# hir0shim/singleSpMV

Measured on AMD Instinct MI355X. Metric: SpMV GFLOP/s (fp64) + achieved HBM GB/s, higher is better.
Workload: dtype f64

## Files before the change

singlespmv_amd/csrc/k_bin.hip:

```cpp
#include "device.hpp"
#include "internal.hpp"

namespace spmv {

typedef uint32_t bin_u32x4 __attribute__((ext_vector_type(4)));

template <int U>
struct MulBatch {
    double v[U];
    uint32_t c[U];
    int32_t d[U];
};

template <int U, int PL, int MODE, bool LONG>
__device__ __forceinline__ void mul_load(MulBatch<U> &B, int64_t base, int64_t e0, int64_t e1, int lane,
                                         const double *__restrict__ val1, const uint16_t *__restrict__ cs1,
                                         const int32_t *__restrict__ dst1, int64_t ls, int64_t lsh,
                                         const int32_t *__restrict__ lcode) {
    if constexpr (!LONG) {
        const double *vb = val1 + base + lane;
        const uint16_t *cb = cs1 + base + lane;
        const int32_t *db = dst1 + ((base + lane) >> PL);
#pragma unroll
        for (int u = 0; u < U; ++u) {
            B.v[u] = ld_stream(vb + u * 64);
            B.c[u] = (uint32_t)__builtin_nontemporal_load(cb + u * 64);
            if constexpr ((MODE & 4) == 0) B.d[u] = ld_stream(db + u * (64 >> PL));
        }
        (void)e0;
        (void)e1;
        (void)ls;
        (void)lsh;
        (void)lcode;
        (void)db;
    } else {
#pragma unroll
        for (int u = 0; u < U; ++u) {
            const int64_t e = base + u * 64 + lane;
            const int64_t ee = e < e1 ? e : e0;
            B.v[u] = ld_stream(val1 + ee);
            B.c[u] = (uint32_t)__builtin_nontemporal_load(cs1 + ee);
            if (base + u * 64 >= ls) B.d[u] = ld_stream(lcode + (e < e1 ? e + lsh : 0));
            else if constexpr ((MODE & 4) == 0) B.d[u] = ld_stream(dst1 + (ee >> PL));
        }
    }
}

__device__ __forceinline__ void mul_long_block(double pr, int32_t code, bool ok, int lane,
                                               double *__restrict__ prod) {
    const bool start = code < 0 || !ok;
    const uint64_t starts = __ballot(start);
    const uint64_t upto = starts & (~0ull >> (63 - lane));
    const int seg = 63 - __clzll((long long)upto);
    const int r16 = lane & 15, row = lane >> 4;
    double v = ok ? pr : 0.0, t;
    t = dpp_f64<0x111, 0xF>(v);
    if (r16 >= 1 && lane - 1 >= seg) v = __dadd_rn(t, v);
    t = dpp_f64<0x112, 0xF>(v);
    if (r16 >= 2 && lane - 2 >= seg) v = __dadd_rn(t, v);
    t = dpp_f64<0x114, 0xF>(v);
    if (r16 >= 4 && lane - 4 >= seg) v = __dadd_rn(t, v);
    t = dpp_f64<0x118, 0xF>(v);
    if (r16 >= 8 && lane - 8 >= seg) v = __dadd_rn(t, v);
    t = dpp_f64<0x142, 0xA>(v);
    if ((row & 1) && seg <= row * 16 - 1) v = __dadd_rn(t, v);
    t = dpp_f64<0x143, 0xC>(v);
    if (row >= 2 && seg <= 31) v = __dadd_rn(t, v);
    const int32_t pos = code & 0x7FFFFFFF;
    if (ok && pos != 0x7FFFFFFF) prod[pos] = v;
}

template <int U, int MODE, int PL, bool LONG>
__device__ __forceinline__ void mul_store(const MulBatch<U> &B, int64_t base, int64_t e1, int lane,
                                          const double *xs, double *__restrict__ prod, int64_t ls) {
#pragma unroll
    for (int u = 0; u < U; ++u) {
        const int64_t e = base + u * 64 + lane;
        if (LONG && base + u * 64 >= ls) {
            mul_long_block(__dmul_rn(B.v[u], xs[B.c[u]]), B.d[u], e < e1, lane, prod);
        } else if (e < e1) {
            const double pr = __dmul_rn(B.v[u], xs[B.c[u]]);
            double *dp = (MODE & 4) ? prod + e : prod + ((int64_t)B.d[u] << PL) + (e & ((1 << PL) - 1));
            if (MODE & 1) __builtin_nontemporal_store(pr, dp);
            else *dp = pr;
        }
    }
}

template <int U, int MODE, int PL, bool LONG>
__global__ __launch_bounds__(kBinMulThreads) void bin_mul_kernel(
    const int64_t *__restrict__ piece_off, int64_t q_base, const int32_t *__restrict__ piece_strip,
    const int64_t *__restrict__ piece_begin, const int64_t *__restrict__ piece_end,
    const double *__restrict__ val1, const uint16_t *__restrict__ cs1, const int32_t *__restrict__ dst1,
    const double *__restrict__ x, int64_t n, int32_t strip, double *__restrict__ prod,
    const int64_t *__restrict__ lstart, const int64_t *__restrict__ lshift, const int32_t *__restrict__ lcode,
    int32_t xburst) {
    __shared__ double xs[kBinMaxStrip];
    constexpr int NW = kBinMulThreads / 64;
    constexpr int64_t STEP = (int64_t)NW * 64 * U;
    const int w = __builtin_amdgcn_readfirstlane(threadIdx.x >> 6);
    const int lane = threadIdx.x & 63;
    const int64_t q0 = piece_off[q_base + blockIdx.x], q1 = piece_off[q_base + blockIdx.x + 1];
    for (int64_t q = q0; q < q1; ++q) {
        const int32_t st = piece_strip[q];
        const int64_t c0 = (int64_t)st * strip;
        const int64_t e0 = piece_begin[q], e1 = piece_end[q];
        const int64_t ls = LONG ? lstart[st] : INT64_MAX, lsh = LONG ? lshift[st] : 0;
        const int cw = (int)(n - c0 < strip ? n - c0 : strip);
        __syncthreads();
        constexpr int XL = 8;
        if constexpr ((MODE & 256) != 0) {
            const int full = cw & ~127;
            for (int k = w; k * 128 < full; k += NW)
                __builtin_amdgcn_global_load_lds(
                    (const __attribute__((address_space(1))) void *)(x + c0 + k * 128 + lane * 2),
                    (__attribute__((address_space(3))) void *)(xs + k * 128), 16, 0, 0);
            for (int i = full + threadIdx.x; i < cw; i += kBinMulThreads) xs[i] = x[c0 + i];
            __builtin_amdgcn_s_waitcnt(0x0F70);
        } else if (LONG || !xburst) {
            for (int i = threadIdx.x; i < cw; i += kBinMulThreads) xs[i] = x[c0 + i];
        } else for (int i0 = threadIdx.x; i0 < cw; i0 += XL * kBinMulThreads) {
            double t[XL];
#pragma unroll
            for (int k = 0; k < XL; ++k) {
                const int i = i0 + k * kBinMulThreads;
                t[k] = i < cw ? x[c0 + i] : 0.0;
            }
#pragma unroll
            for (int k = 0; k < XL; ++k) {
                const int i = i0 + k * kBinMulThreads;
                if (i < cw) xs[i] = t[k];
            }
        }
        __syncthreads();
        const int64_t first = e0 + (int64_t)w * 64 * U;
        const int64_t nit = first < e1 ? (e1 - first + STEP - 1) / STEP : 0;
        auto bat = [&](int64_t j) { return first + j * STEP; };
        MulBatch<U> A, B;
        if (nit > 0) mul_load<U, PL, MODE, LONG>(A, bat(0), e0, e1, lane, val1, cs1, dst1, ls, lsh, lcode);
        for (int64_t it = 0; it < nit; it += 2) {
            const int64_t ba = bat(it), bb = bat(it + 1);
            if (it + 1 < nit) mul_load<U, PL, MODE, LONG>(B, bb, e0, e1, lane, val1, cs1, dst1, ls, lsh, lcode);
            mul_store<U, MODE, PL, LONG>(A, ba, e1, lane, xs, prod, ls);
            if (it + 1 < nit) {
                if (it + 2 < nit)
                    mul_load<U, PL, MODE, LONG>(A, bat(it + 2), e0, e1, lane, val1, cs1, dst1, ls, lsh, lcode);
                mul_store<U, MODE, PL, LONG>(B, bb, e1, lane, xs, prod, ls);
            }
        }
    }
}

template <int U>
struct SumBatch {
    double v[U];
    uint32_t w[U / 2];
    __device__ __forceinline__ uint32_t slot(int u) const { return (w[u >> 1] >> (16 * (u & 1))) & 0xFFFFu; }
};

template <int U>
__device__ __forceinline__ void sum_load(SumBatch<U> &B, int64_t base, int lane, int64_t pbase, int64_t sbase,
                                         const uint16_t *__restrict__ slot2, const double *__restrict__ prod) {
    static_assert(U % 8 == 0, "slots are read 8 per 16-byte load");
    const bin_u32x4 *sp = reinterpret_cast<const bin_u32x4 *>(slot2 + sbase + (int64_t)lane * 8);
#pragma unroll
    for (int q = 0; q < U / 8; ++q) {
        const bin_u32x4 w = __builtin_nontemporal_load(sp + q * 64);
#pragma unroll
        for (int h = 0; h < 4; ++h) B.w[4 * q + h] = w[h];
    }
    const double *pp = prod + (base - pbase) + lane;
#pragma unroll
    for (int u = 0; u < U; ++u) B.v[u] = ld_stream(pp + u * 64);
}

template <int U>
__device__ __forceinline__ void sum_add(const SumBatch<U> &B, double *ys) {
#pragma unroll
    for (int u = 0; u < U; ++u) atomicAdd(&ys[B.slot(u)], B.v[u]);
}

template <int W2, int U>
__global__ __launch_bounds__(64 * W2) void bin_sum_kernel(
    int64_t b0, int64_t b1, int64_t nbins, int64_t nblk, const int64_t *__restrict__ run_off,
    const int64_t *__restrict__ srun_off, const int32_t *__restrict__ bin_row0, int64_t pbase,
    const uint16_t *__restrict__ slot2,
    const double *__restrict__ prod, double *__restrict__ y) {
    constexpr int SLICE = kBinLdsDoubles / W2;
    constexpr int64_t STEP = 64 * U;
    __shared__ double ylds[kBinLdsDoubles];
    const int w = __builtin_amdgcn_readfirstlane(threadIdx.x >> 6);
    const int lane = threadIdx.x & 63;
    double *ys = ylds + w * SLICE;
    const int64_t bfirst = b0 + (int64_t)blockIdx.x * W2 + w, bstride = (int64_t)gridDim.x * W2;
    if (bfirst >= b1) return;
    int64_t cb = bfirst, k = 0, pos = run_off[cb], end = run_off[cb + 1], rs = pos, ss = srun_off[cb];
    auto next = [&](int64_t &lo, int64_t &sb, int64_t &bb) -> bool {
        while (pos >= end) {
            if (++k >= nblk) {
                cb += bstride;
                if (cb >= b1) return false;
                k = 0;
                pos = rs = run_off[cb];
                end = run_off[cb + 1];
                ss = srun_off[cb];
                continue;
            }
            pos = rs = run_off[k * nbins + cb];
            end = run_off[k * nbins + cb + 1];
            ss = srun_off[k * nbins + cb];
        }
        lo = pos;
        sb = ss + (lo - rs);
        bb = cb;
        pos = pos + STEP < end ? pos + STEP : end;
        return true;
    };
    int64_t acc = -1, done = bfirst;
    auto write_zero = [&](int64_t bz) {
        const int64_t r0 = bin_row0[bz];
        const int rows = (int)(bin_row0[bz + 1] - r0);
        for (int i = lane; i < rows; i += 64) __builtin_nontemporal_store(0.0, y + r0 + i);
    };
    auto finish = [&]() {
        const int64_t r0 = bin_row0[acc];
        const int rows = (int)(bin_row0[acc + 1] - r0);
        __builtin_amdgcn_fence(__ATOMIC_SEQ_CST, "wavefront");
        for (int i = lane; i < rows; i += 64) __builtin_nontemporal_store(ys[i], y + r0 + i);
        __builtin_amdgcn_fence(__ATOMIC_SEQ_CST, "wavefront");
        done = acc + bstride;
    };
    auto begin = [&](int64_t nb) {
        if (nb == acc) return;
        if (acc >= 0) finish();
        for (; done < nb; done += bstride) write_zero(done);
        const int rows = (int)(bin_row0[nb + 1] - bin_row0[nb]);
        for (int i = lane; i < rows; i += 64) ys[i] = 0.0;
        acc = nb;
        done = nb + bstride;
    };
    SumBatch<U> A, B;
    int64_t alo, asb, ab, blo, bsb, bbn;
    bool has_a = next(alo, asb, ab);
    if (has_a) sum_load<U>(A, alo, lane, pbase, asb, slot2, prod);
    while (has_a) {
        const bool has_b = next(blo, bsb, bbn);
        if (has_b) sum_load<U>(B, blo, lane, pbase, bsb, slot2, prod);
        begin(ab);
        sum_add<U>(A, ys);
        if (!has_b) break;
        has_a = next(alo, asb, ab);
        if (has_a) sum_load<U>(A, alo, lane, pbase, asb, slot2, prod);
        begin(bbn);
        sum_add<U>(B, ys);
    }
    if (acc >= 0) finish();
    for (; done < b1; done += bstride) write_zero(done);
}

template <int U>
struct SumTab {
    int32_t t[U / 8];
};

template <int U>
__device__ __forceinline__ void sum_mo_tab(SumTab<U> &T, int64_t sb, int lane, const int32_t *__restrict__ mtab) {
    static_assert(U == 32, "U/8 = 4 table words per lane: one 16-byte load");
    const bin_u32x4 w = __builtin_nontemporal_load(reinterpret_cast<const bin_u32x4 *>(mtab + (sb >> 3)) + lane);
#pragma unroll
    for (int h = 0; h < 4; ++h) T.t[h] = (int32_t)w[h];
}

template <int U>
__device__ __forceinline__ void sum_mo_load(SumBatch<U> &B, const SumTab<U> &T, int64_t sb, int lane,
                                            const uint16_t *__restrict__ slot2, const double *__restrict__ prod) {
    const bin_u32x4 *sp = reinterpret_cast<const bin_u32x4 *>(slot2 + sb + (int64_t)lane * 8);
#pragma unroll
    for (int q = 0; q < U / 8; ++q) {
        const bin_u32x4 w = __builtin_nontemporal_load(sp + q * 64);
#pragma unroll
        for (int h = 0; h < 4; ++h) B.w[4 * q + h] = w[h];
    }
    const double *pl = prod + (lane & 7);
    int c[U];
#pragma unroll
    for (int u = 0; u < U; ++u) c[u] = __builtin_amdgcn_ds_bpermute((((u & 7) << 3) + (lane >> 3)) << 2, T.t[u >> 3]);
    __builtin_amdgcn_sched_barrier(0);
#pragma unroll
    for (int u = 0; u < U; ++u) B.v[u] = pl[c[u]];
}

template <int W2, int U>
__global__ __launch_bounds__(64 * W2) void bin_sum_bin_kernel(
    int64_t b0, int64_t b1, const int64_t *__restrict__ run_off, const int64_t *__restrict__ srun_off,
    const int32_t *__restrict__ bin_row0, const uint16_t *__restrict__ slot2, const int32_t *__restrict__ mtab,
    const double *__restrict__ prod, double *__restrict__ y) {
    constexpr int SLICE = kBinLdsDoubles / W2;
    constexpr int64_t STEP = 64 * U;
    __shared__ double ylds[kBinLdsDoubles];
    const int w = __builtin_amdgcn_readfirstlane(threadIdx.x >> 6);
    const int lane = threadIdx.x & 63;
    double *ys = ylds + w * SLICE;
    struct BinRun {
        int64_t r0 = 0, nb = 0, ss0 = 0;
        int rows = 0;
        __device__ int64_t s(int64_t j) const { return ss0 + j * STEP; }
    };
    auto bin_at = [&](int64_t b) {
        BinRun R;
        R.r0 = bin_row0[b];
        R.rows = (int)(bin_row0[b + 1] - R.r0);
        R.ss0 = srun_off[b];
        R.nb = (run_off[b + 1] - run_off[b] + STEP - 1) / STEP;
        return R;
    };
    const int64_t bstride = (int64_t)gridDim.x * W2;
    int64_t b = b0 + (int64_t)blockIdx.x * W2 + w;
    if (b >= b1) return;
    BinRun R = bin_at(b);
    for (int i = lane; i < R.rows; i += 64) ys[i] = 0.0;
    SumBatch<U> PA, PB;
    SumTab<U> TA, TB;
    bool pre = false;
    for (;;) {
        const int64_t bn = b + bstride;
        const bool more = bn < b1;
        const BinRun N = more ? bin_at(bn) : R;
        const bool pfn = more && N.nb > 0;
        auto sbat = [&](int64_t j) -> int64_t {
            if (j < R.nb) return R.s(j);
            return pfn ? N.s(j - R.nb < N.nb ? j - R.nb : N.nb - 1) : R.s(R.nb - 1);
        };
        bool swapped = false;
        if (R.nb > 0) {
            if (!pre) {
                sum_mo_tab<U>(TA, sbat(0), lane, mtab);
                sum_mo_tab<U>(TB, sbat(1), lane, mtab);
                sum_mo_load<U>(PA, TA, sbat(0), lane, slot2, prod);
            } else if (R.nb == 1) {
                sum_mo_tab<U>(TB, sbat(1), lane, mtab);
            }
            for (int64_t j = 0;; j += 2) {
                sum_mo_tab<U>(TA, sbat(j + 2), lane, mtab);
                sum_mo_load<U>(PB, TB, sbat(j + 1), lane, slot2, prod);
                sum_add<U>(PA, ys);
                if (j + 1 >= R.nb) {
                    swapped = true;
                    break;
                }
                sum_mo_tab<U>(TB, sbat(j + 3), lane, mtab);
                sum_mo_load<U>(PA, TA, sbat(j + 2), lane, slot2, prod);
                sum_add<U>(PB, ys);
                if (j + 2 >= R.nb) break;
            }
        }
        pre = R.nb > 0 && pfn;
        __builtin_amdgcn_fence(__ATOMIC_SEQ_CST, "wavefront");
        for (int i = lane; i < R.rows; i += 64) __builtin_nontemporal_store(ys[i], y + R.r0 + i);
        __builtin_amdgcn_fence(__ATOMIC_SEQ_CST, "wavefront");
        if (!more) break;
        for (int i = lane; i < N.rows; i += 64) ys[i] = 0.0;
        if (pre && swapped) {
            PA = PB;
            TB = TA;
        }
        b = bn;
        R = N;
    }
}

template <int W2>
static void launch_sum_mo(const spmv_plan_s *p, double *y) {
    const BinDev &B = p->bin;
    hipLaunchKernelGGL((bin_sum_bin_kernel<W2, 32>), dim3((unsigned)B.nwg2), dim3(64 * W2), 0, p->stream,
                       (int64_t)0, B.n_bins, B.run_off, B.srun_off, B.bin_row0, B.slot2, B.mtab, B.prod, y);
}

template <int MODE, int PL, int U = 8>
static void launch_mul_t(const spmv_plan_s *p, int g, const double *x) {
    const BinDev &B = p->bin;
    if (B.long_len > 0)
        hipLaunchKernelGGL((bin_mul_kernel<U, MODE, PL, true>), dim3((unsigned)B.nwg1), dim3(kBinMulThreads), 0,
                           p->stream, B.piece_off, (int64_t)g * B.nwg1, B.piece_strip, B.piece_begin, B.piece_end,
                           B.val1, B.cs1, B.dst1, x, p->n, (int32_t)B.strip, B.prod, B.lstart, B.lshift, B.lcode,
                           B.xburst);
    else
        hipLaunchKernelGGL((bin_mul_kernel<U, MODE, PL, false>), dim3((unsigned)B.nwg1), dim3(kBinMulThreads), 0,
                           p->stream, B.piece_off, (int64_t)g * B.nwg1, B.piece_strip, B.piece_begin, B.piece_end,
                           B.val1, B.cs1, B.dst1, x, p->n, (int32_t)B.strip, B.prod, nullptr, nullptr, nullptr,
                           B.xburst);
}

template <int PL>
static void launch_mul_p(const spmv_plan_s *p, int g, const double *x) {
    bool dma = (reinterpret_cast<uintptr_t>(x) & 15) == 0 && p->bin.strip % 2 == 0;
    if (launch_dbg(p->bin.dbg) & (1 << 24)) dma = false;
    if (p->bin.mo) {
        if (dma) launch_mul_t<256 | 4, PL>(p, g, x);
        else launch_mul_t<4, PL>(p, g, x);
    } else {
        if (dma) launch_mul_t<256 | 1, PL>(p, g, x);
        else launch_mul_t<1, PL>(p, g, x);
    }
}

static void launch_mul(const spmv_plan_s *p, int g, const double *x) {
    if (p->bin.pad_log == 5) launch_mul_p<5>(p, g, x);
    else if (p->bin.pad_log == 4) launch_mul_p<4>(p, g, x);
    else launch_mul_p<3>(p, g, x);
}

template <int W2, int U>
static void launch_sum_w(const spmv_plan_s *p, int g, double *y) {
    const BinDev &B = p->bin;
    const int64_t b0 = g < 0 ? 0 : B.g_bin[g], b1 = g < 0 ? B.n_bins : B.g_bin[g + 1];
    const int64_t pbase = g < 0 ? 0 : B.g_prod[g];
    hipLaunchKernelGGL((bin_sum_kernel<W2, U>), dim3((unsigned)B.nwg2), dim3(64 * W2), 0, p->stream, b0, b1,
                       B.n_bins, B.n_blocks, B.run_off, B.srun_off, B.bin_row0, pbase, B.slot2, B.prod, y);
}

int bin_time_mul(const spmv_plan_s *p, const double *x, float *ms) {
    const BinDev &B = p->bin;
    hipEvent_t a, b;
    SPMV_HIP_TRY(hipEventCreate(&a));
    SPMV_HIP_TRY(hipEventCreate(&b));
    for (int rep = 0; rep < 2; ++rep) {
        if (rep == 1) SPMV_HIP_TRY(hipEventRecord(a, p->stream));
        for (int g = 0; g < B.G; ++g) {
            launch_mul(p, g, x);
        }
    }
    SPMV_HIP_TRY(hipEventRecord(b, p->stream));
    SPMV_HIP_TRY(hipEventSynchronize(b));
    SPMV_HIP_TRY(hipEventElapsedTime(ms, a, b));
    (void)hipEventDestroy(a);
    (void)hipEventDestroy(b);
    return SPMV_SUCCESS;
}

int launch_bin(const spmv_plan_s *p, const double *x, double *y) {
    const BinDev &B = p->bin;
    if (p->m == 0) return SPMV_SUCCESS;
    if (p->nnz == 0) {
        SPMV_HIP_TRY(hipMemsetAsync(y, 0, sizeof(double) * (size_t)p->m, p->stream));
        return SPMV_SUCCESS;
    }
    auto sum = [&](int g) {
        if (B.mo) {
            if (B.sum_waves == 2) launch_sum_mo<2>(p, y);
            else launch_sum_mo<4>(p, y);
            return;
        }
        if (B.sum_waves == 2) launch_sum_w<2, 32>(p, g, y);
        else if (B.sum_waves == 4) launch_sum_w<4, 32>(p, g, y);
        else launch_sum_w<8, 8>(p, g, y);
    };
    for (int g = 0; g < B.G; ++g) {
        launch_mul(p, g, x);
        SPMV_HIP_TRY(hipGetLastError());
        if (B.reuse) {
            phase_mark(p);
            sum(g);
            SPMV_HIP_TRY(hipGetLastError());
            if (g + 1 < B.G) phase_mark(p);
        }
    }
    if (!B.reuse) {
        phase_mark(p);
        sum(-1);
        SPMV_HIP_TRY(hipGetLastError());
    }
    return SPMV_SUCCESS;
}

}
```

Baseline: 396.4.

## Add team mode to bin sum kernel sharing one LDS bin across waves

Restructures the bin sum kernel so that, for the 2-wave configuration, P waves form a team working on one bin with a single LDS slice. The waves take turns applying atomic adds while the others prefetch their next batch, and the per-bin index tables are read through the constant address space. The aim is to overlap loads with LDS accumulation and to raise the number of resident workgroups by shrinking LDS per block. The cost is a workgroup barrier every turn, plus serialised adds within each team. The 4-wave setting keeps the old per-wave path (P=1), and probe flags allow switching between variants.

After: 396.7 (median of 3 runs). About the same (+0.1%).

```diff
diff --git a/singlespmv_amd/csrc/k_bin.hip b/singlespmv_amd/csrc/k_bin.hip
--- a/singlespmv_amd/csrc/k_bin.hip
+++ b/singlespmv_amd/csrc/k_bin.hip
@@ -180,22 +180,17 @@
     for (int u = 0; u < U; ++u) atomicAdd(&ys[B.slot(u)], B.v[u]);
 }
 
-template <int W2, int U>
-__global__ __launch_bounds__(64 * W2) void bin_sum_kernel(
-    int64_t b0, int64_t b1, int64_t nbins, int64_t nblk, const int64_t *__restrict__ run_off,
-    const int64_t *__restrict__ srun_off, const int32_t *__restrict__ bin_row0, int64_t pbase,
-    const uint16_t *__restrict__ slot2,
-    const double *__restrict__ prod, double *__restrict__ y) {
-    constexpr int SLICE = kBinLdsDoubles / W2;
-    constexpr int64_t STEP = 64 * U;
-    __shared__ double ylds[kBinLdsDoubles];
-    const int w = __builtin_amdgcn_readfirstlane(threadIdx.x >> 6);
-    const int lane = threadIdx.x & 63;
-    double *ys = ylds + w * SLICE;
-    const int64_t bfirst = b0 + (int64_t)blockIdx.x * W2 + w, bstride = (int64_t)gridDim.x * W2;
-    if (bfirst >= b1) return;
-    int64_t cb = bfirst, k = 0, pos = run_off[cb], end = run_off[cb + 1], rs = pos, ss = srun_off[cb];
-    auto next = [&](int64_t &lo, int64_t &sb, int64_t &bb) -> bool {
+template <typename TAB>
+struct SumCursor {
+    TAB run_off, srun_off;
+    int64_t nbins, nblk, b1, bstride;
+    int64_t cb, k, pos, end, rs, ss;
+    __device__ __forceinline__ SumCursor(TAB ro, TAB so, int64_t nbins_, int64_t nblk_, int64_t bfirst, int64_t b1_,
+                                         int64_t bstride_)
+        : run_off(ro), srun_off(so), nbins(nbins_), nblk(nblk_), b1(b1_), bstride(bstride_), cb(bfirst), k(0),
+          pos(ro[bfirst]), end(ro[bfirst + 1]), rs(pos), ss(so[bfirst]) {}
+    template <int64_t STEP>
+    __device__ __forceinline__ bool next(int64_t &lo, int64_t &sb, int64_t &bb) {
         while (pos >= end) {
             if (++k >= nblk) {
                 cb += bstride;
@@ -215,8 +210,90 @@
         bb = cb;
         pos = pos + STEP < end ? pos + STEP : end;
         return true;
-    };
+    }
+};
+
+template <int W2, int U, int P>
+__global__ __launch_bounds__(64 * (P == 1 ? W2 : P)) void bin_sum_kernel(
+    int64_t b0, int64_t b1, int64_t nbins, int64_t nblk, const int64_t *__restrict__ run_off,
+    const int64_t *__restrict__ srun_off, const int32_t *__restrict__ bin_row0, int64_t pbase,
+    const uint16_t *__restrict__ slot2,
+    const double *__restrict__ prod, double *__restrict__ y) {
+    constexpr int SLICE = kBinLdsDoubles / W2;
+    constexpr int64_t STEP = 64 * U;
+    __shared__ double ylds[P == 1 ? kBinLdsDoubles : SLICE];
+    const int w = __builtin_amdgcn_readfirstlane(threadIdx.x >> 6);
+    const int lane = threadIdx.x & 63;
+    double *ys = P == 1 ? ylds + w * SLICE : ylds;
+    const int64_t bfirst = b0 + (P == 1 ? (int64_t)blockIdx.x * W2 + w : (int64_t)blockIdx.x);
+    const int64_t bstride = (int64_t)gridDim.x * (P == 1 ? W2 : 1);
+    if (bfirst >= b1) return;
     int64_t acc = -1, done = bfirst;
+    if constexpr (P > 1) {
+        typedef const __attribute__((address_space(4))) int64_t *ctab;
+        const SumCursor<ctab> first((ctab)run_off, (ctab)srun_off, nbins, nblk, bfirst, b1, bstride);
+        SumCursor<ctab> step = first, mine = first;
+        constexpr int T = 64 * P;
+        const int tid = threadIdx.x;
+        auto team_barrier = [&]() {
+            __builtin_amdgcn_fence(__ATOMIC_SEQ_CST, "wavefront");
+            __builtin_amdgcn_s_waitcnt(0xC07F);
+            __builtin_amdgcn_s_barrier();
+            __builtin_amdgcn_fence(__ATOMIC_SEQ_CST, "wavefront");
+        };
+        auto zero_rows = [&](int64_t bz) {
+            const int64_t r0 = bin_row0[bz];
+            const int rows = (int)(bin_row0[bz + 1] - r0);
+            for (int i = tid; i < rows; i += T) __builtin_nontemporal_store(0.0, y + r0 + i);
+        };
+        auto write_back = [&]() {
+            const int64_t r0 = bin_row0[acc];
+            const int rows = (int)(bin_row0[acc + 1] - r0);
+            for (int i0 = tid; i0 < rows; i0 += 4 * T) {
+                double v[4];
+#pragma unroll
+                for (int q = 0; q < 4; ++q) v[q] = i0 + q * T < rows ? ys[i0 + q * T] : 0.0;
+#pragma unroll
+                for (int q = 0; q < 4; ++q)
+                    if (i0 + q * T < rows) __builtin_nontemporal_store(v[q], y + r0 + i0 + q * T);
+            }
+            done = acc + bstride;
+        };
+        SumBatch<U> A;
+        auto load_mine = [&](int skip) {
+            int64_t lo, sb, bb;
+            bool has = true;
+#pragma unroll
+            for (int i = 0; i < P - 1; ++i)
+                if (i < skip && has) has = mine.template next<STEP>(lo, sb, bb);
+            if (has && mine.template next<STEP>(lo, sb, bb)) sum_load<U>(A, lo, lane, pbase, sb, slot2, prod);
+        };
+        load_mine(w);
+        int turn = 0;
+        int64_t lo, sb, nb;
+        while (step.template next<STEP>(lo, sb, nb)) {
+            if (nb != acc) {
+                if (acc >= 0) write_back();
+                for (; done < nb; done += bstride) zero_rows(done);
+                const int rows = (int)(bin_row0[nb + 1] - bin_row0[nb]);
+                for (int i = tid; i < rows; i += T) ys[i] = 0.0;
+                acc = nb;
+                done = nb + bstride;
+                team_barrier();
+            }
+            if (turn == w) {
+                sum_add<U>(A, ys);
+                load_mine(P - 1);
+            }
+            team_barrier();
+            turn = turn + 1 == P ? 0 : turn + 1;
+        }
+        if (acc >= 0) write_back();
+        for (; done < b1; done += bstride) zero_rows(done);
+        return;
+    }
+    SumCursor<const int64_t *> cur(run_off, srun_off, nbins, nblk, bfirst, b1, bstride);
+    auto next = [&](int64_t &lo, int64_t &sb, int64_t &bb) -> bool { return cur.template next<STEP>(lo, sb, bb); };
     auto write_zero = [&](int64_t bz) {
         const int64_t r0 = bin_row0[bz];
         const int rows = (int)(bin_row0[bz + 1] - r0);
@@ -410,13 +487,36 @@
     else launch_mul_p<3>(p, g, x);
 }
 
-template <int W2, int U>
+template <int W2, int U, int P>
 static void launch_sum_w(const spmv_plan_s *p, int g, double *y) {
     const BinDev &B = p->bin;
     const int64_t b0 = g < 0 ? 0 : B.g_bin[g], b1 = g < 0 ? B.n_bins : B.g_bin[g + 1];
     const int64_t pbase = g < 0 ? 0 : B.g_prod[g];
-    hipLaunchKernelGGL((bin_sum_kernel<W2, U>), dim3((unsigned)B.nwg2), dim3(64 * W2), 0, p->stream, b0, b1,
-                       B.n_bins, B.n_blocks, B.run_off, B.srun_off, B.bin_row0, pbase, B.slot2, B.prod, y);
+    const unsigned grid = (unsigned)(P == 1 ? B.nwg2 : B.nwg2 * W2), block = 64 * (P == 1 ? W2 : P);
+#ifdef SPMV_PROBES
+    if (probe_env("SPMV_BIN_SUM_OCCUPANCY")) {
+        static bool said = false;
+        int nb = -1;
+        if (!said && hipOccupancyMaxActiveBlocksPerMultiprocessor(&nb, bin_sum_kernel<W2, U, P>, (int)block, 0) ==
+                         hipSuccess)
+            std::fprintf(stderr, "bin_sum_kernel<%d, %d, %d>: block %u, %d workgroups per CU\n", W2, U, P, block, nb);
+        said = true;
+    }
+#endif
+    hipLaunchKernelGGL((bin_sum_kernel<W2, U, P>), dim3(grid), dim3(block), 0, p->stream, b0, b1, B.n_bins,
+                       B.n_blocks, B.run_off, B.srun_off, B.bin_row0, pbase, B.slot2, B.prod, y);
+}
+
+constexpr int kBinSumTeam2 = 2, kBinSumTeam2Alt = 4, kBinSumTeam4 = 1, kBinSumTeam4Alt = 2;
+
+template <int W2, int U, int P, int ALT>
+static void launch_sum_p(const spmv_plan_s *p, int g, double *y) {
+#ifdef SPMV_PROBES
+    const int dbg = launch_dbg(p->bin.dbg);
+    if (dbg & (1 << 25)) return launch_sum_w<W2, U, 1>(p, g, y);
+    if (dbg & (1 << 26)) return launch_sum_w<W2, U, ALT>(p, g, y);
+#endif
+    launch_sum_w<W2, U, P>(p, g, y);
 }
 
 int bin_time_mul(const spmv_plan_s *p, const double *x, float *ms) {
@@ -451,9 +551,9 @@
             else launch_sum_mo<4>(p, y);
             return;
         }
-        if (B.sum_waves == 2) launch_sum_w<2, 32>(p, g, y);
-        else if (B.sum_waves == 4) launch_sum_w<4, 32>(p, g, y);
-        else launch_sum_w<8, 8>(p, g, y);
+        if (B.sum_waves == 2) launch_sum_p<2, 32, kBinSumTeam2, kBinSumTeam2Alt>(p, g, y);
+        else if (B.sum_waves == 4) launch_sum_p<4, 32, kBinSumTeam4, kBinSumTeam4Alt>(p, g, y);
+        else launch_sum_w<8, 8, 1>(p, g, y);
     };
     for (int g = 0; g < B.G; ++g) {
         launch_mul(p, g, x);
```
